# LPMP/BDD

Hardware: AMD Instinct MI355X
Metric: parallel-MMA iterations/sec, 10.5M BDD nodes, 1 GPU (+ achieved HBM GB/s in roofline) (higher is better)
Workload: dtype f32

## Files before the change

bdd_amd/capi.py:

```python
from __future__ import annotations

import ctypes as C
import os
import subprocess

_HERE = os.path.dirname(os.path.abspath(__file__))
LIB_PATH = os.path.abspath(os.environ["BDDMMA_LIB"]) if os.environ.get("BDDMMA_LIB") else os.path.join(_HERE, "csrc", "libbdd_mma_hip.so")

OK = 0
ERR_INVALID_ARGUMENT, ERR_INVALID_BDD, ERR_DEVICE, ERR_STATE, ERR_UNSUPPORTED, ERR_IO = -1, -2, -3, -4, -5, -6
F32, F64 = 0, 1
K_FORWARD_MM, K_BACKWARD_MM, K_FINISH_DELTA, K_OTHER, K_COUNT = 0, 1, 2, 3, 4


class Options(C.Structure):
    _fields_ = [("pack_width", C.c_uint32), ("wide_pack_width", C.c_uint32), ("deterministic", C.c_uint32),
                ("vars_per_bin", C.c_uint32), ("stage_cap", C.c_uint32), ("waves_per_block", C.c_uint32),
                ("keep_bdd_order", C.c_uint32), ("resident_sweeps", C.c_uint32), ("exchange_by_variable", C.c_uint32),
                ("variant_flags", C.c_uint32), ("pack_fill", C.c_uint32), ("pack_stagger", C.c_uint32)]


class LbfgsParams(C.Structure):
    _fields_ = [("history_size", C.c_int32), ("init_step_size", C.c_double), ("req_rel_lb_increase", C.c_double),
                ("step_size_decrease_factor", C.c_double), ("step_size_increase_factor", C.c_double)]
# ... 25 lines not shown
    "bddmma_last_error": (C.c_char_p, [_V]),
    "bddmma_nr_variables": (_U64, [_V]),
    "bddmma_nr_bdds": (_U64, [_V]),
    "bddmma_nr_layers": (_U64, [_V]),
    "bddmma_nr_bdd_nodes": (_U64, [_V]),
    "bddmma_nr_hops": (_U64, [_V]),
    "bddmma_nr_packs": (_U64, [_V]),
    "bddmma_solve_sweep_kind": (_I, [_V]),
    "bddmma_fused_small": (_I, [_V]),
    "bddmma_fused_small_learned": (_I, [_V]),
    "bddmma_fused_small_history": (_I, [_V]),
    "bddmma_fused_small_stop": (_I, [_V]),
    "bddmma_nontemporal_loads": (_I, [_V]),
    "bddmma_potentials_on_chip": (_I, [_V]),
    "bddmma_onchip_hops": (_I, [_V]),
    "bddmma_precision": (_I, [_V]),
    "bddmma_device": (_I, [_V]),
    "bddmma_num_bdds_per_var": (_I, [_V, _V]),
    "bddmma_layer_variables": (_I, [_V, _V]),
    "bddmma_layer_bdds": (_I, [_V, _V]),
    "bddmma_nodes_per_hop": (_I, [_V, _V]),
    "bddmma_layers_per_hop": (_I, [_V, _V]),
    "bddmma_update_costs": (_I, [_V, _V, _U64, _V, _U64, _I, _I]),
    "bddmma_set_cost": (_I, [_V, _D, _U64]),
    "bddmma_get_solver_costs": (_I, [_V, _V, _V, _V, _I]),
    "bddmma_set_solver_costs": (_I, [_V, _V, _V, _V, _I]),
    "bddmma_primal_objective_vec": (_I, [_V, _V, _I]),
    "bddmma_forward_run": (_I, [_V]),
    "bddmma_backward_run": (_I, [_V]),
    "bddmma_lower_bound": (_I, [_V, C.POINTER(_D)]),
# ... 70 lines not shown
    "bddmma_stream_signal": (_I, [_V, _V]),
    "bddmma_set_profiling": (_I, [_V, _I]),
    "bddmma_get_profile": (_I, [_V, C.POINTER(Profile)]),
    "bddmma_time_iterations": (_I, [_V, _D, _U64, C.POINTER(_D)]),
    "bddmma_time_kernel": (_I, [_V, _I, _U64, C.POINTER(_D)]),
    "bddmma_device_bytes": (_U64, [_V]),
    "bddmma_device_allocated_bytes": (_U64, [_V]),
    "bddmma_layout_create": (_I, [C.POINTER(_V), _V, _V, _U64, C.POINTER(Options)]),
    "bddmma_layout_create_for_chip": (_I, [C.POINTER(_V), _V, _V, _U64, C.POINTER(Options), _I, C.c_uint32, C.c_uint32]),
    "bddmma_layout_destroy": (None, [_V]),
    "bddmma_layout_size": (_U64, [_V, _I]),
    "bddmma_layout_copy": (_I, [_V, _I, _V]),
    "bddmma_layout_res2_records": (_I, [_V, _I, _V, _V, _V]),
    "bddmma_layout_stream_records": (_I, [_V, _I, _V, _V, _V]),
    "bddmma_layout_layer_records": (_I, [_V, _I, _V, _V, _V]),
    "bddmma_layout_seg_exchange": (_I, [_V, _I, _I, _V, _V, _V, _V]),
}

_I64P, _U64P = C.POINTER(C.c_int64), C.POINTER(C.c_uint64)
ILP_SIGNATURES = {
    "bddilp_last_error": (C.c_char_p, []),
    "bddilp_parse_lp": (_I, [C.c_char_p, C.POINTER(_V)]),
    "bddilp_parse_opb": (_I, [C.c_char_p, C.POINTER(_V)]),
    "bddilp_parse": (_I, [C.c_char_p, C.POINTER(_V)]),
    "bddilp_destroy": (None, [_V]),
    "bddilp_nr_variables": (_U64, [_V]),
    "bddilp_nr_constraints": (_U64, [_V]),
    "bddilp_variable_name": (C.c_char_p, [_V, _U64]),
    "bddilp_objective": (_I, [_V, _V, C.POINTER(_D)]),
    "bddilp_constraint_size": (_U64, [_V, _U64]),
# ... 53 lines not shown
```

bdd_amd/csrc/capi.cpp:

```cpp
#include <chrono>
#include <cmath>
#include <cstdio>
#include <cstdlib>
#include <cstring>
#include <limits>
#include <new>
#include <string>
#include <vector>

#include "../../include/bdd_mma.h"
#include "layout.hpp"
#include "solver.hpp"

using namespace bddmma;

struct bddmma_lbfgs;
extern "C" int bddmma_lbfgs_iteration(bddmma_lbfgs* l);
extern "C" int bddmma_lbfgs_update_costs(bddmma_lbfgs* l, const void* lo, uint64_t n_lo, const void* hi, uint64_t n_hi, int elem_precision,
                                         int on_device);

namespace {
thread_local std::string g_err;

template <typename F>
// ... 121 lines not shown

uint64_t bddmma_nr_variables(const bddmma_solver* s) { return s && s->impl ? s->impl->n_vars : 0; }
uint64_t bddmma_nr_bdds(const bddmma_solver* s) { return s && s->impl ? s->impl->n_bdds : 0; }
uint64_t bddmma_nr_layers(const bddmma_solver* s) { return s && s->impl ? s->impl->n_layers : 0; }
uint64_t bddmma_nr_bdd_nodes(const bddmma_solver* s) { return s && s->impl ? s->impl->n_input_nodes : 0; }
uint64_t bddmma_nr_hops(const bddmma_solver* s) { return s && s->impl ? s->impl->n_hops : 0; }
uint64_t bddmma_nr_packs(const bddmma_solver* s) { return s && s->impl ? s->impl->n_packs_narrow + s->impl->n_packs_wide : 0; }
int bddmma_solve_sweep_kind(const bddmma_solver* s) { return s && s->impl ? s->impl->solve_sweep_kind : -1; }
int bddmma_fused_small(const bddmma_solver* s) { return s && s->impl ? (s->impl->fused_small ? 1 : 0) : -1; }
int bddmma_fused_small_learned(const bddmma_solver* s) { return s && s->impl ? (s->impl->fused_small_learned ? 1 : 0) : -1; }
int bddmma_fused_small_history(const bddmma_solver* s) { return s && s->impl ? (s->impl->fused_small_history ? 1 : 0) : -1; }
int bddmma_fused_small_stop(const bddmma_solver* s) { return s && s->impl ? (s->impl->fused_small_stop ? 1 : 0) : -1; }
int bddmma_nontemporal_loads(const bddmma_solver* s) { return s && s->impl ? (s->impl->nt_loads ? 1 : 0) : -1; }
int bddmma_potentials_on_chip(const bddmma_solver* s) { return s && s->impl ? (s->impl->pot_on_chip ? 1 : 0) : -1; }
int bddmma_onchip_hops(const bddmma_solver* s) { return s && s->impl ? s->impl->onchip_hops : -1; }
int bddmma_precision(const bddmma_solver* s) { return s && s->impl ? s->impl->precision : -1; }
int bddmma_device(const bddmma_solver* s) { return s && s->impl ? s->impl->device : -1; }
uint64_t bddmma_device_bytes(const bddmma_solver* s) { return s && s->impl ? s->impl->dev_bytes : 0; }
uint64_t bddmma_device_allocated_bytes(const bddmma_solver* s) { return s && s->impl ? s->impl->dev_alloc_bytes : 0; }

int bddmma_num_bdds_per_var(const bddmma_solver* s, int32_t* out)
{
    return guarded(s, [&](SolverBase* b) { return copy_host(b->h_nbdds, out); });
}
int bddmma_layer_variables(const bddmma_solver* s, int32_t* out)
{
    return guarded(s, [&](SolverBase* b) { return copy_host(b->h_layer_var, out); });
}
int bddmma_layer_bdds(const bddmma_solver* s, int32_t* out)
{
// ... 786 lines not shown
    if (rec_off && !R.rec_off.empty()) std::memcpy(rec_off, R.rec_off.data(), R.rec_off.size() * sizeof(uint32_t));
    return BDDMMA_OK;
}

int bddmma_layout_layer_records(const bddmma_layout* l, int real_size, uint32_t* info, uint32_t* words, uint32_t* rec_off)
{
    if (!l || !info || (real_size != 4 && real_size != 8)) return BDDMMA_ERR_INVALID_ARGUMENT;
    LayerRecords R;
    build_layer_records(l->L, (uint32_t)real_size, R);
    info[0] = R.ok ? 1u : 0u; info[1] = (uint32_t)R.rec.size();
    if (words && !R.rec.empty()) std::memcpy(words, R.rec.data(), R.rec.size() * sizeof(uint32_t));
    if (rec_off && !R.rec_off.empty()) std::memcpy(rec_off, R.rec_off.data(), R.rec_off.size() * sizeof(uint32_t));
    return BDDMMA_OK;
}

}
```

bdd_amd/csrc/kernels.hpp:

```cpp
#pragma once
#include <hip/hip_runtime.h>

#include <cstdint>
#include <type_traits>

#include "layout.hpp"

#include "kernels/common.hpp"
#include "kernels/stream.hpp"
#include "kernels/narrow.hpp"
#include "kernels/resident.hpp"
#include "kernels/narrow2.hpp"
#include "kernels/narrow3.hpp"
#include "kernels/narrow4.hpp"
#include "kernels/wide.hpp"
#include "kernels/exchange.hpp"
#include "kernels/small.hpp"
#include "kernels/elementwise.hpp"
```

bdd_amd/csrc/layout.cpp:

```cpp
#include "layout.hpp"

#include <algorithm>
#include <atomic>
#include <chrono>
#include <cstdio>
#include <cstdlib>
#include <mutex>
#include <thread>
#include <unordered_map>
#include <cstring>
#include <limits>

namespace bddmma {

namespace {

std::atomic<unsigned> g_layout_threads{0};
thread_local unsigned t_layout_threads = 0;
struct Par {
    unsigned nt = 1;
    Par()
    {
        const char* e = std::getenv("BDDMMA_THREADS");
        const unsigned hw = std::thread::hardware_concurrency();
// ... 1562 lines not shown
                    ++l;
                } else {
                    if (pos != 1 || l == 0 || !(w & NW_TWO) || (r[4 * (l - 1) + 2] & 0xFFFFu) != (j - 1) * S) { out = LayerRecords(); return; }
                    const uint32_t k = l - 1;
                    r[4 * k + 1] = child(lo, k) | (child(hi, k) << 16);
                    r[4 * k + 2] |= LREC_TWO << 16;
                    r[4 * k + 3] = (r[4 * k + 3] & 0xFFFFu) | ((j * S) << 16);
                }
            }
            if (l != nl) { out = LayerRecords(); return; }
        }
    }
    out.ok = true;
}

void set_layout_threads(unsigned n) { g_layout_threads.store(n, std::memory_order_relaxed); }
void set_thread_layout_threads(unsigned n) { t_layout_threads = n; }

}
```

bdd_amd/csrc/layout.hpp:

```cpp
#pragma once
#include <cstdint>
#include <string>
#include <vector>

#include "../../include/bdd_mma.h"

#ifndef __host__
#define __host__
#define __device__
#endif

namespace bddmma {

constexpr uint32_t NW_CHILD_BITS = 9;
constexpr uint32_t NW_CHILD_MASK = (1u << NW_CHILD_BITS) - 1;
constexpr uint32_t NW_POS_SHIFT = 18, NW_LIDX_SHIFT = 24, NW_FIELD6 = 63;
constexpr uint32_t NW_TWO = 1u << 30;
constexpr uint32_t NW_PAD = 1u << 31;
constexpr uint32_t nw_top(uint32_t pack_width) { return pack_width; }
constexpr uint32_t nw_bot(uint32_t pack_width) { return pack_width + 1; }
constexpr uint32_t nw_pad_word(uint32_t pack_width)
{
    return NW_PAD | (nw_bot(pack_width) << NW_CHILD_BITS) | nw_bot(pack_width);
}
// ... 166 lines not shown
    bool ok = false;
    std::vector<uint32_t> rec;
    std::vector<uint32_t> rec_off;
};
void build_stream_records(const HostLayout& L, uint32_t real_size, StreamRecords& out);

constexpr uint32_t LREC_NO_STORE = 0xFFF0u;
constexpr uint32_t LREC_TWO = 1u, LREC_REAL = 2u;
struct LayerRecords {
    bool ok = false;
    std::vector<uint32_t> rec;
    std::vector<uint32_t> rec_off;
};
void build_layer_records(const HostLayout& L, uint32_t real_size, LayerRecords& out);

struct LinComb {
    const char* g;
    const void* S;
    const char* Y;
    uint64_t slot;
    const double* cy;
    const double* cs;
    const uint32_t* order;
    int ns;
};
constexpr int LINCOMB_MAX = 8;

struct SegExchange {
    bool ok = false;
    uint32_t threads = 0;
// ... 20 lines not shown
```

bdd_amd/csrc/solver.hpp:

```cpp
#pragma once
#include <hip/hip_runtime.h>

#include <cstdint>
#include <limits>
#include <memory>
#include <string>
#include <utility>
#include <vector>

#include "../../include/bdd_mma.h"
#include "layout.hpp"

namespace bddmma {

struct SolverBase {
    int precision = BDDMMA_F32, device = -1;
    hipStream_t stream = nullptr;
    std::string err;
    uint64_t n_vars = 0, n_bdds = 0, n_layers = 0, n_hops = 0, n_input_nodes = 0, n_slots = 0;
    int solve_sweep_kind = 0;
    uint32_t pack_width = 0, wide_pack_width = 0, wide_slot_base = 0;
    uint64_t dev_bytes = 0;
    uint64_t dev_alloc_bytes = 0;
    bool fwd_valid = false, bwd_valid = false;
// ... 34 lines not shown
        return BDDMMA_OK;
    }
    virtual int learned_iterations(const void* dist_weights, int weights_on_device, uint64_t num_itr, double omega, double improvement_slope,
                                   void* sol_avg, void* lb_first_diff_avg, void* lb_second_diff_avg, uint64_t compute_history_for_itr,
                                   double history_avg_beta, int outputs_on_device, uint64_t* itr_done, const void* omega_vec,
                                   int omega_vec_on_device) = 0;
    virtual int isotropic_dist_weights(void* out, int on_device) = 0;
    double initial_lb_change = std::numeric_limits<double>::infinity();
    std::shared_ptr<int> lbfgs_attached = std::make_shared<int>(0);
    bool fused_small = false;
    bool fused_small_learned = false;
    bool fused_small_history = false;
    bool fused_small_stop = false;
    bool nt_loads = false;
    bool pot_on_chip = false;
    int onchip_hops = 0;
    virtual int run_plain(uint64_t max_iter, double tolerance, double slope, double time_limit, int verbose, bddmma_run_result* res) = 0;
    virtual int forward_mm(double omega, void* delta, int on_device) = 0;
    virtual int backward_mm(double omega, void* delta, int on_device) = 0;
    virtual int normalize_delta(void* delta, int on_device) = 0;
    virtual int distribute_delta() = 0;
    virtual int get_delta(void* out, int on_device) = 0;
    virtual int set_delta(const void* in, int on_device) = 0;
    virtual int update_costs(const void* lo, uint64_t n_lo, const void* hi, uint64_t n_hi, int elem_precision, int on_device) = 0;
    virtual int set_cost(double c, uint64_t var) = 0;
    virtual int get_solver_costs(void* lo, void* hi, void* mm, int on_device) = 0;
    virtual int set_solver_costs(const void* lo, const void* hi, const void* mm, int on_device) = 0;
    virtual int primal_objective_vec(void* out, int on_device) = 0;
    virtual int min_marginals(int sorted, int32_t* var, void* mm0, void* mm1, int on_device) = 0;
    virtual int min_marginal_diff(void* out, int on_device) = 0;
// ... 92 lines not shown
```

bdd_amd/csrc/solver_impl.hpp:

```cpp
#pragma once
#include <hip/hip_runtime.h>
#include <atomic>
#include <chrono>
#include <cmath>
#include <cstdio>
#include <cstdlib>
#include <cstring>
#include <limits>
#include <memory>
#include <string>
#include <thread>
#include <type_traits>
#include <vector>
#include "../../include/bdd_mma.h"
#include "kernels.hpp"
#include "layout.hpp"
#include "solver.hpp"

namespace bddmma {

static inline void cpu_relax()
{
#if defined(__x86_64__) || defined(__i386__)
    __asm__ __volatile__("pause");
// ... 132 lines not shown
    int small_nw = 1;
    uint32_t small_lds = 0;
    SmallDev small{};
    uint32_t* d_small_lds = nullptr;
    bool small_ln_ok = false, small_ln_rl = false, sl_ready = false;
    bool small_stop_ok = false;
    bool small_hist_ok = false;
    uint32_t small_ln_lds = 0;
    SmallDev small_ln{};
    SmallLearn<REAL> small_ln_arg{};
    bool use_narrow3 = false;
    int onchip_hc = 0;
    uint32_t onchip_mode = 0;
    uint32_t *d_lrec = nullptr, *d_lrec_off = nullptr;
    uint32_t lrec_words = 0;
    uint32_t huge_pack_width = 0;
    unsigned char* d_huge_scratch = nullptr;

    std::vector<void*> allocs;

    ~SolverT() override
    {
        if (device >= 0) (void)hipSetDevice(device);
        for (void* p : allocs) (void)hipFree(p);
        if (h_lb) (void)hipHostFree(h_lb);
        if (h_lb_seq) (void)hipHostFree(h_lb_seq);
        if (h_run) (void)hipHostFree(h_run);
        if (d_run_ctl) (void)hipFree(d_run_ctl);
        for (auto& e : ev_pool) {
            (void)hipEventDestroy(e.first);
// ... 257 lines not shown
                const uint64_t in_flight = (uint64_t)n_cus * wgs2 * wpb;
                const bool auto_ok = sizeof(REAL) == 4 ? (uint64_t)nb_.n_packs * 100 <= in_flight * 145 : (uint64_t)nb_.n_packs <= in_flight;
                if (wgs2 && (mode == 2 || auto_ok)) {
                    Res2Records R2;
                    build_res2_records(L, sizeof(REAL), res2_ns, res2_nl, R2);
                    if (R2.ok && R2.rec.size() * sizeof(uint32_t) < (1ull << 31)) {
                        if ((rc = upload(&d_res2_rec, R2.rec))) return rc;
                        if ((rc = upload(&d_res2_rec_off, R2.rec_off))) return rc;
                        res2_n_words = (uint32_t)R2.rec.size();
                        use_res2 = use_res = true;
                    }
                }
            }
        }
        uint32_t narrow2_static = 0;
        if (nb_.n_packs && !use_res && !wb_.n_packs && !(opts && (opts->variant_flags & 0x1000u))) {
            StreamRecords SR;
            build_stream_records(L, sizeof(REAL), SR);
            narrow2_static = L.ex.waves_per_block * ((2 * pack_width + 2 + pack_width + 2) * (uint32_t)sizeof(REAL) + 3 * 64 * 4 + 64);
            const bool forced = opts && (opts->variant_flags & 0x2000u);
            const bool shared = forced || (SR.rec.size() * sizeof(uint32_t) <= (uint64_t)L.narrow_slots * sizeof(REAL) / 2 &&
                                           (sizeof(REAL) == 8 || n_slots <= 16'000'000ull));
            if (SR.ok && shared && stage_lds + narrow2_static + seg_bytes(L.ex.waves_per_block) <= 64 * 1024) {
                if ((rc = upload(&d_srec, SR.rec))) return rc;
                if ((rc = upload(&d_srec_off, SR.rec_off))) return rc;
                srec_words = (uint32_t)SR.rec.size();
                use_narrow2 = true;
                narrow_gen = narrow_seg;
                for (uint16_t r : L.narrow.hop_root) narrow_gen = narrow_gen || r != NO_ROOT;
            }
        }
        if (nb_.n_packs && !use_res && !wb_.n_packs && !hb_.n_packs && !narrow_seg && pack_width == 128 && (L.ex.waves_per_block == 4 || L.ex.waves_per_block == 8) &&
            !(opts && (opts->variant_flags & 0x41000u))) {
            LayerRecords LR;
            build_layer_records(L, sizeof(REAL), LR);
            const uint32_t n3_static = L.ex.waves_per_block * (4 * (128 + 128) * (uint32_t)sizeof(REAL) + 3 * 64 * 4);
            const bool forced = opts && (opts->variant_flags & 0x2000u);
            const bool shared = forced || (LR.rec.size() * sizeof(uint32_t) <= (uint64_t)L.narrow_slots * sizeof(REAL) / 2 && n_slots <= 16'000'000ull);
            if (LR.ok && shared && stage_lds + n3_static <= lds_cu - 1024) {
                if ((rc = upload(&d_lrec, LR.rec))) return rc;
                if ((rc = upload(&d_lrec_off, LR.rec_off))) return rc;
                lrec_words = (uint32_t)LR.rec.size();
                use_narrow3 = true;
                n3_nt = sizeof(REAL) == 8 && nt_potentials != 0;
            }
        }
        if (nb_.n_packs && !use_res && !use_narrow3 && !wb_.n_packs && !hb_.n_packs && !narrow_seg && !narrow_gen && pack_width == 128 &&
            (L.ex.waves_per_block == 4 || L.ex.waves_per_block == 8) && (beyond_cache || (opts && (opts->variant_flags & 0x100000u))))
#ifndef BDDMMA_EXP_NO_N12_NT
            n12_nt = !use_narrow2 || sizeof(REAL) == 8;
// ... 2 lines not shown
#endif
        nt_loads = n3_nt || n12_nt;
        if constexpr (sizeof(REAL) == 4) {
            if (use_narrow3 && res_hdr_ok && !n3_nt && !(opts && (opts->variant_flags & 0x200000u))) {
                uint32_t max_hops = 0;
                for (uint32_t p = 0; p < nb_.n_packs; ++p) max_hops = std::max(max_hops, L.res.pack_hdr[8 * (size_t)p + 5] & 0xFFFFu);
                onchip_hc = max_hops <= 10 ? 10 : max_hops <= 12 ? 12 : max_hops <= 16 ? 16 : 0;
                const uint32_t part = opts ? (opts->variant_flags >> 22) & 3u : 0u;
                if (onchip_hc == 16) onchip_mode = 3;
                if (part == 1 || part == 2) {
                    if (onchip_hc == 10 && wpb == 4) onchip_mode = part;
                    else onchip_hc = 0;
                }
                pot_on_chip = onchip_hc != 0;
                onchip_hops = onchip_hc;
            }
        }
        if (wb_.n_packs) {
            wide_threads = std::min<uint32_t>(1024, std::max<uint32_t>(64, ((wide_pack_width + 1) / 2 + 63) / 64 * 64));
            wide_npt = (wide_pack_width + wide_threads - 1) / wide_threads;
            wide_npt = wide_npt <= 1 ? 1 : (wide_npt <= 2 ? 2 : 4);
            wide_lds = (uint32_t)wide2_lds_bytes(sizeof(REAL), wide_pack_width, true);
            if (wide_lds > lds_cu || wide_pack_width > 4096) {
                err = "wide_pack_width " + std::to_string(wide_pack_width) + " needs " + std::to_string(wide_lds) + " B of LDS (> 160 KiB)";
                return BDDMMA_ERR_UNSUPPORTED;
            }
        }
        if (wb_.n_packs && nb_.n_packs && !use_res && !(opts && (opts->variant_flags & 1u))) {
            const uint32_t threads = 64 * wpb;
            const uint32_t npt = (wide_pack_width + threads - 1) / threads;
// ... 189 lines not shown
            if (mixed)
                s.mixed = {pick<64, 128, 256>(pack_width, [&](auto PW) {
                               return pick<1, 2, 4, 8>(wpb, [&](auto W) {
                                   return pick<1, 2, 4>(mixed_npt, [&](auto N) -> MixedFn {
                                       constexpr int R = PW.value / 64;
                                       return bwd ? &k_bwd_mixed<REAL, R, W.value, N.value, OV> : &k_fwd_mixed<REAL, R, W.value, N.value, OV>;
                                   });
                               });
                           }),
                           mixed_lds};
        }
        return s;
    }
    RecFn onchip_fn(bool bwd, bool rebuild, bool store) const
    {
        if (onchip_hc == 16) return pick<4, 8>(wpb, [&](auto W) -> RecFn { return &k_bwd_narrow4<REAL, W.value, 16, true, true>; });
        if (onchip_hc == 12)
            return pick<4, 8>(wpb, [&](auto W) -> RecFn {
                return bwd ? &k_bwd_narrow4<REAL, W.value, 12, true, false> : &k_fwd_narrow4<REAL, W.value, 12, true, false>;
            });
        if (rebuild && !store)
            return pick<4, 8>(wpb, [&](auto W) -> RecFn {
                return bwd ? &k_bwd_narrow4<REAL, W.value, 10, true, false> : &k_fwd_narrow4<REAL, W.value, 10, true, false>;
            });
        if (rebuild) return bwd ? &k_bwd_narrow4<REAL, 4, 10, true, true> : &k_fwd_narrow4<REAL, 4, 10, true, true>;
        return bwd ? &k_bwd_narrow4<REAL, 4, 10, false, false> : &k_fwd_narrow4<REAL, 4, 10, false, false>;
    }
    void resolve_kernels()
    {
        for (int bwd = 0; bwd < 2; ++bwd) {
            kern.sweep[bwd][FWD_PLAIN] = resolve_sweep<FWD_PLAIN, false>(bwd);
            kern.sweep[bwd][FWD_SOLVE] = resolve_sweep<FWD_SOLVE, false>(bwd);
            kern.sweep[bwd][FWD_SOLUTION] = resolve_sweep<FWD_SOLUTION, false>(bwd);
        }
        if (onchip_hc) {
            for (int bwd = 0; bwd < 2; ++bwd) {
                Sweep s = kern.sweep[bwd][FWD_SOLVE];
                if (onchip_mode == 3 && !bwd) { kern.onchip[0] = s; continue; }
                const bool rebuild = onchip_mode == 0 || (onchip_mode == 1) == !bwd;
                const bool store = onchip_mode != 0 && rebuild;
                if constexpr (sizeof(REAL) == 4) s.rec = onchip_fn(bwd, rebuild, onchip_mode == 3 || store);
                s.reads_pot = !rebuild;
                s.stores_pot = onchip_mode == 3 || store;
                kern.onchip[bwd] = s;
            }
        }
        kern.ex_threads = exch_small ? EXS_THREADS : exch_medium ? EXM_THREADS : EX_THREADS;
        pick<EXS_THREADS, EXM_THREADS, EX_THREADS>(kern.ex_threads, [&](auto T_) {
            constexpr int T = T_.value, U = T == EXS_THREADS ? EXS_UNROLL : T == EXM_THREADS ? EXM_UNROLL : EX_UNROLL,
                          N = T == EXS_THREADS ? EXS_NPT : T == EXM_THREADS ? EXM_NPT : EX_NPT;
            kern.ex[0] = {&k_exchange_reduce<REAL, BDDMMA_EX_ACC, EX_ITER, T, U, N, false>, exch_lds};
            kern.ex[1] = {&k_exchange_reduce<REAL, BDDMMA_EX_ACC, EX_ITER, T, U, N, true>, exch_lds};
            kern.ex_w = {&k_exchange_reduce<REAL, BDDMMA_EX_ACC, EX_ITER, T, U, N, false, true>, exch_lds};
            kern.project = {&k_project_entries<REAL, T>, vars_per_bin * (uint32_t)sizeof(double)};
            if (use_seg)
                pick<2, 4>(seg_groups <= 2 ? 2 : 4, [&](auto G) {
// ... 1265 lines not shown
```

bdd_amd/solver.py:

```python
from __future__ import annotations

import ctypes as C

import numpy as np

from . import capi
from .bdd_collection import BddCollection


def _ptr(a):
    return a.ctypes.data_as(C.c_void_p) if a is not None else None


def _is_dev(x):
    return hasattr(x, "data_ptr") and bool(getattr(x, "is_cuda", False))


def _dev_ptr(x, n, dtype):
    assert x.is_contiguous() and x.numel() >= n, "device buffer too small or not contiguous"
    assert x.element_size() == np.dtype(dtype).itemsize, "device buffer has the wrong element type"
    return C.c_void_p(x.data_ptr())


class bdd_hip_parallel_mma:
# ... 53 lines not shown
    def fused_small_learned(self) -> bool:
        return bool(self._L.bddmma_fused_small_learned(self._h))
    def fused_small_history(self) -> bool:
        return bool(self._L.bddmma_fused_small_history(self._h))
    def fused_small_stop(self) -> bool:
        return bool(self._L.bddmma_fused_small_stop(self._h))

    def nontemporal_loads(self) -> bool:
        return bool(self._L.bddmma_nontemporal_loads(self._h))

    def potentials_on_chip(self) -> bool:
        return bool(self._L.bddmma_potentials_on_chip(self._h))

    def onchip_hops(self) -> int:
        return int(self._L.bddmma_onchip_hops(self._h))
    def device(self) -> int:
        return int(self._L.bddmma_device(self._h))
    def device_bytes(self): return int(self._L.bddmma_device_bytes(self._h))
    def device_allocated_bytes(self): return int(self._L.bddmma_device_allocated_bytes(self._h))

    def nr_bdds(self, var=None):
        if var is None:
            return int(self._L.bddmma_nr_bdds(self._h))
        return int(self.get_num_bdds_per_var()[var])

    def get_num_bdds_per_var(self):
        out = np.zeros(self.nr_variables(), np.int32)
        self._ck(self._L.bddmma_num_bdds_per_var(self._h, _ptr(out)))
        return out

# ... 797 lines not shown
```

include/bdd_mma.h:

```cpp
#ifndef BDD_MMA_H
#define BDD_MMA_H

#include <stddef.h>
#include <stdint.h>

#ifdef __cplusplus
extern "C" {
#endif

#define BDDMMA_OK 0
#define BDDMMA_ERR_INVALID_ARGUMENT (-1)
#define BDDMMA_ERR_INVALID_BDD (-2)
#define BDDMMA_ERR_DEVICE (-3)
#define BDDMMA_ERR_STATE (-4)
#define BDDMMA_ERR_UNSUPPORTED (-5)
#define BDDMMA_ERR_IO (-6)

#define BDDMMA_F32 0
#define BDDMMA_F64 1

typedef struct bddmma_instruction {
    uint64_t lo;
    uint64_t hi;
    uint64_t index;
// ... 42 lines not shown
    BDDMMA_SWEEPS_MIXED = 1,
    BDDMMA_SWEEPS_STREAMING1 = 2,
    BDDMMA_SWEEPS_STREAMING2 = 3,
    BDDMMA_SWEEPS_STREAMING3 = 4,
    BDDMMA_SWEEPS_RESIDENT1 = 5,
    BDDMMA_SWEEPS_RESIDENT2 = 6
};
int bddmma_solve_sweep_kind(const bddmma_solver* s);
int bddmma_fused_small(const bddmma_solver* s);
int bddmma_fused_small_learned(const bddmma_solver* s);
int bddmma_fused_small_history(const bddmma_solver* s);
int bddmma_fused_small_stop(const bddmma_solver* s);
int bddmma_nontemporal_loads(const bddmma_solver* s);
int bddmma_potentials_on_chip(const bddmma_solver* s);
int bddmma_onchip_hops(const bddmma_solver* s);
int bddmma_precision(const bddmma_solver* s);
int bddmma_device(const bddmma_solver* s);
int bddmma_num_bdds_per_var(const bddmma_solver* s, int32_t* out);
int bddmma_layer_variables(const bddmma_solver* s, int32_t* out);
int bddmma_layer_bdds(const bddmma_solver* s, int32_t* out);
int bddmma_nodes_per_hop(const bddmma_solver* s, uint64_t* out);
int bddmma_layers_per_hop(const bddmma_solver* s, uint64_t* out);

int bddmma_update_costs(bddmma_solver* s, const void* lo, uint64_t n_lo, const void* hi, uint64_t n_hi,
                        int elem_precision, int on_device);
int bddmma_set_cost(bddmma_solver* s, double c, uint64_t var);
int bddmma_get_solver_costs(const bddmma_solver* s, void* lo, void* hi, void* deferred_mm_diff, int on_device);
int bddmma_set_solver_costs(bddmma_solver* s, const void* lo, const void* hi, const void* deferred_mm_diff, int on_device);
int bddmma_primal_objective_vec(bddmma_solver* s, void* out, int on_device);

// ... 159 lines not shown
int bddmma_time_kernel(bddmma_solver* s, int kind, uint64_t reps, double* ms);
uint64_t bddmma_device_bytes(const bddmma_solver* s);
uint64_t bddmma_device_allocated_bytes(const bddmma_solver* s);

typedef struct bddmma_layout bddmma_layout;
int bddmma_layout_create(bddmma_layout** out, const bddmma_instruction* instr, const uint64_t* bdd_delims,
                         uint64_t n_bdds, const bddmma_options* opts);
int bddmma_layout_create_for_chip(bddmma_layout** out, const bddmma_instruction* instr, const uint64_t* bdd_delims,
                                  uint64_t n_bdds, const bddmma_options* opts, int real_size, uint32_t n_cus, uint32_t lds_bytes_per_cu);
void bddmma_layout_destroy(bddmma_layout* l);
uint64_t bddmma_layout_size(const bddmma_layout* l, int what);
int bddmma_layout_copy(const bddmma_layout* l, int which, void* out);
int bddmma_layout_res2_records(const bddmma_layout* l, int real_size, uint32_t* info, uint32_t* words, uint32_t* rec_off);
int bddmma_layout_stream_records(const bddmma_layout* l, int real_size, uint32_t* info, uint32_t* words, uint32_t* rec_off);
int bddmma_layout_layer_records(const bddmma_layout* l, int real_size, uint32_t* info, uint32_t* words, uint32_t* rec_off);
int bddmma_layout_seg_exchange(const bddmma_layout* l, int threads, int real_size, uint32_t* info, uint32_t* bin, uint16_t* perm, uint32_t* thr);

#ifdef __cplusplus
}
#endif
#endif
```

Measured before the change: 9727.

## Add lane-code on-chip sweep kernels encoding per-lane child topology in compact bit codes

Adds a new narrow5 forward/backward kernel that replaces per-hop layer record tables with a compact 10-bit per-hop, per-lane code (packed three hops per 32-bit word, one 128-bit load per lane). Each code says whether a child is the next layer's node A/B, the top sink or the bottom sink. The kernels resolve children with bit-select arithmetic instead of LDS-indexed gathers. The host builds and deduplicates these codes, and the path is enabled only for f32 when on-chip hop counts are 10 or 12 in mode 0. It cuts record traffic and LDS indexing in exchange for extra ALU bit manipulation and more host-side layout complexity.

Result: faster. 9891 (median of 6 runs) (+1.7%).

```diff
diff --git a/bdd_amd/capi.py b/bdd_amd/capi.py
--- a/bdd_amd/capi.py
+++ b/bdd_amd/capi.py
@@ -63,6 +63,7 @@
     "bddmma_nontemporal_loads": (_I, [_V]),
     "bddmma_potentials_on_chip": (_I, [_V]),
     "bddmma_onchip_hops": (_I, [_V]),
+    "bddmma_lane_sweeps": (_I, [_V]),
     "bddmma_precision": (_I, [_V]),
     "bddmma_device": (_I, [_V]),
     "bddmma_num_bdds_per_var": (_I, [_V, _V]),
@@ -163,6 +164,7 @@
     "bddmma_layout_res2_records": (_I, [_V, _I, _V, _V, _V]),
     "bddmma_layout_stream_records": (_I, [_V, _I, _V, _V, _V]),
     "bddmma_layout_layer_records": (_I, [_V, _I, _V, _V, _V]),
+    "bddmma_layout_lane_codes": (_I, [_V, _I, _V, _V, _V]),
     "bddmma_layout_seg_exchange": (_I, [_V, _I, _I, _V, _V, _V, _V]),
 }
 
diff --git a/bdd_amd/csrc/capi.cpp b/bdd_amd/csrc/capi.cpp
--- a/bdd_amd/csrc/capi.cpp
+++ b/bdd_amd/csrc/capi.cpp
@@ -159,6 +159,7 @@
 int bddmma_nontemporal_loads(const bddmma_solver* s) { return s && s->impl ? (s->impl->nt_loads ? 1 : 0) : -1; }
 int bddmma_potentials_on_chip(const bddmma_solver* s) { return s && s->impl ? (s->impl->pot_on_chip ? 1 : 0) : -1; }
 int bddmma_onchip_hops(const bddmma_solver* s) { return s && s->impl ? s->impl->onchip_hops : -1; }
+int bddmma_lane_sweeps(const bddmma_solver* s) { return s && s->impl ? (s->impl->lane_sweeps ? 1 : 0) : -1; }
 int bddmma_precision(const bddmma_solver* s) { return s && s->impl ? s->impl->precision : -1; }
 int bddmma_device(const bddmma_solver* s) { return s && s->impl ? s->impl->device : -1; }
 uint64_t bddmma_device_bytes(const bddmma_solver* s) { return s && s->impl ? s->impl->dev_bytes : 0; }
@@ -975,4 +976,17 @@
     return BDDMMA_OK;
 }
 
-}
+int bddmma_layout_lane_codes(const bddmma_layout* l, int real_size, uint32_t* info, uint32_t* words, uint32_t* code_off)
+{
+    if (!l || !info || (real_size != 4 && real_size != 8)) return BDDMMA_ERR_INVALID_ARGUMENT;
+    LayerRecords R;
+    build_layer_records(l->L, (uint32_t)real_size, R);
+    LaneCodes K;
+    build_lane_codes(l->L, (uint32_t)real_size, R, K);
+    info[0] = K.ok ? 1u : 0u; info[1] = (uint32_t)K.words.size(); info[2] = K.affine ? 1u : 0u;
+    if (words && !K.words.empty()) std::memcpy(words, K.words.data(), K.words.size() * sizeof(uint32_t));
+    if (code_off && !K.code_off.empty()) std::memcpy(code_off, K.code_off.data(), K.code_off.size() * sizeof(uint32_t));
+    return BDDMMA_OK;
+}
+
+}
diff --git a/bdd_amd/csrc/kernels.hpp b/bdd_amd/csrc/kernels.hpp
--- a/bdd_amd/csrc/kernels.hpp
+++ b/bdd_amd/csrc/kernels.hpp
@@ -13,6 +13,7 @@
 #include "kernels/narrow2.hpp"
 #include "kernels/narrow3.hpp"
 #include "kernels/narrow4.hpp"
+#include "kernels/narrow5.hpp"
 #include "kernels/wide.hpp"
 #include "kernels/exchange.hpp"
 #include "kernels/small.hpp"
diff --git a/bdd_amd/csrc/kernels/narrow5.hpp b/bdd_amd/csrc/kernels/narrow5.hpp
--- /dev/null
+++ b/bdd_amd/csrc/kernels/narrow5.hpp
@@ -0,0 +1,261 @@
+#pragma once
+
+namespace bddmma {
+
+#ifndef BDDMMA_N5_WAVES
+#define BDDMMA_N5_WAVES 5
+#endif
+constexpr int n5_waves(int hc) { return hc <= 10 ? BDDMMA_N5_WAVES : 4; }
+
+__device__ __forceinline__ uint32_t lane_hop_code(const u4v& cw, int h) { return (cw[h / 3] >> (10 * (h % 3))) & 0x3FFu; }
+__device__ __forceinline__ u4v lane_codes_again(const u4v& cw)
+{
+    uint32_t a = cw[0], b = cw[1], c = cw[2], e = cw[3];
+    asm volatile("" : "+v"(a), "+v"(b), "+v"(c), "+v"(e));
+    return u4v{a, b, c, e};
+}
+__device__ __forceinline__ uint32_t lane_bit(uint32_t code, uint32_t bit) { return (uint32_t)__builtin_amdgcn_sbfe((int)code, bit, 1u); }
+__device__ __forceinline__ float lane_pick(uint32_t m, float a, float b)
+{
+    return __builtin_bit_cast(float, (m & __builtin_bit_cast(uint32_t, a)) | (~m & __builtin_bit_cast(uint32_t, b)));
+}
+__device__ __forceinline__ float lane_child(uint32_t code, uint32_t k, float ta, float tb)
+{
+    const uint32_t odd = lane_bit(code, k), snk = lane_bit(code, k + 1);
+    const float node = lane_pick(odd, tb, ta);
+    const float sink = __builtin_bit_cast(float, odd & 0x7F800000u);
+    return lane_pick(snk, sink, node);
+}
+__device__ __forceinline__ void lane_push(float& fa, float& fb, uint32_t code, float p0, float p1, float p2, float p3)
+{
+    const float INF = inf_v<float>();
+    const float pv[4] = {p0, p1, p2, p3};
+    fa = fb = INF;
+#pragma unroll
+    for (uint32_t k = 0; k < 4; ++k) {
+        const uint32_t odd = lane_bit(code, 2 * k), snk = lane_bit(code, 2 * k + 1);
+        fa = rmin(fa, lane_pick(odd | snk, INF, pv[k]));
+        fb = rmin(fb, lane_pick(odd & ~snk, pv[k], INF));
+    }
+}
+
+template <typename REAL, int WPB, int HC>
+__device__ __forceinline__ void fwd_narrow5_body(const DevPtrs<REAL>& d, const PackDev& pk, const uint32_t* __restrict__ lcode,
+                                                 const uint32_t* __restrict__ lcode_off, uint32_t lcode_words, REAL omega, uint32_t block_id)
+{
+    static_assert(HC + 1 <= (int)HOP_WIN, "one window of hop offsets has to hold the pack");
+    static_assert(HC <= (int)LCODE_HOPS, "a lane's code words hold LCODE_HOPS hops");
+    using P2 = typename Pair<REAL>::type;
+    extern __shared__ __attribute__((aligned(16))) unsigned char dyn_lds[];
+    P2* sD = reinterpret_cast<P2*>(dyn_lds);
+    __shared__ uint32_t sOffN_[WPB][HOP_WIN], sOffL_[WPB][HOP_WIN], sOffR_[WPB][HOP_WIN];
+    const uint32_t tid = threadIdx.x;
+    const int wave = __builtin_amdgcn_readfirstlane((int)(tid >> 6));
+    const int lane = tid & 63;
+    const uint32_t n_quads = (pk.n_packs + WPB - 1) / WPB;
+    const uint32_t quad = block_to_pack(block_id, n_quads, pk.xcd_chunk);
+    BDDMMA_EXIT_IF(quad >= n_quads, d)
+    const uint32_t p = quad * WPB + wave;
+    const bool has_pack = p < pk.n_packs;
+    const uint32_t* const hp = pk.hdr_pack + 8 * (size_t)(has_pack ? p : 0);
+    const uint32_t q0 = !has_pack ? 0 : hp[4];
+    const uint32_t hops = !has_pack ? 0 : (hp[5] & 0xFFFFu);
+    const uint32_t q1 = q0 + hops;
+    const uint32_t cbase = has_pack ? lcode_off[p] : 0;
+    const uint32_t c0_h = pk.hdr_quad[4 * (size_t)quad], cnt = pk.hdr_quad[4 * (size_t)quad + 1];
+    BDDMMA_STAMP(p, 0);
+    const REAL INF = inf_v<REAL>();
+    const uint32_t slot_first = !has_pack ? 0 : hp[0], l0 = !has_pack ? 0 : hp[2];
+    NarrowRs<REAL> rs(d);
+    rs.rebase_layers(d, l0);
+    uint32_t ent[STAGE_ITERS], esl[STAGE_ITERS];
+    stage_load_tables<REAL, WPB, BDDMMA_LD_TAB_AUX>(ent, esl, rs, c0_h, cnt, tid);
+    const REAL* const lohi_p = d.lohi + 2 * (size_t)l0;
+    const rsrc_t rc = make_rsrc(lcode, lcode_words);
+    HopWindow hw{sOffN_[wave], sOffL_[wave], sOffR_[wave], q0, q1, slot_first, l0};
+    uint32_t lb[HC + 1];
+    P2 L[HC];
+    P2 T[HC + 1];
+#pragma unroll
+    for (int i = 0; i < HC + 1; ++i) T[i] = P2{REAL(0), REAL(0)};
+    const uint32_t db = (uint32_t)wave * pk.stage_cap * (uint32_t)sizeof(P2);
+    hw.fill(pk, q0, lane);
+#pragma unroll
+    for (int i = 0; i < HC + 1; ++i) lb[i] = hw.layer_off(q0 + i);
+#pragma unroll
+    for (int h = 0; h < HC; ++h)
+        hop_load(L[h], rs.lohi, (uint32_t)h < hops ? (uint32_t)lane * (uint32_t)sizeof(P2) : OOB, lb[h] * (uint32_t)sizeof(P2));
+    u4v cw = __builtin_amdgcn_raw_buffer_load_b128(rc, (uint32_t)lane * 16u, cbase * 16u, 0);
+    {
+        REAL ta = REAL(0), tb = REAL(0);
+#pragma unroll
+        for (int h = HC - 1; h >= 1; --h) {
+            if ((uint32_t)h < hops) {
+                const uint32_t code = lane_hop_code(cw, h);
+                const REAL tla = lane_child(code, 0, ta, tb), tha = lane_child(code, 2, ta, tb);
+                const REAL tlb = lane_child(code, 4, ta, tb), thb = lane_child(code, 6, ta, tb);
+                const P2 c = L[h];
+                ta = rmin(c.y + tha, c.x + tla);
+                tb = rmin(c.y + thb, c.x + tlb);
+                T[h] = P2{ta, tb};
+            }
+        }
+        BDDMMA_STAMP(p, 5);
+    }
+    cw = lane_codes_again(cw);
+    stage_load_pairs<REAL, WPB>(sD, ent, esl, rs, cnt, tid);
+    if (WPB > 1) __syncthreads(); else wave_sync();
+    BDDMMA_STAMP(p, 1);
+    REAL fa = (lane_hop_code(cw, 0) & (LREC_REAL << 8)) ? REAL(0) : INF, fb = INF;
+#pragma unroll
+    for (int h = 0; h < HC; ++h) {
+        if ((uint32_t)h < hops) {
+            const uint32_t code = lane_hop_code(cw, h), flags = code >> 8;
+            const uint32_t lbh = lb[h], lbn = lb[h + 1];
+            const uint32_t stg = db + (lbh + (uint32_t)lane) * (uint32_t)sizeof(P2);
+            const P2 c = L[h];
+            const P2 tn = T[h + 1];
+            const REAL tla = lane_child(code, 0, tn.x, tn.y), tha = lane_child(code, 2, tn.x, tn.y);
+            const REAL tlb = lane_child(code, 4, tn.x, tn.y), thb = lane_child(code, 6, tn.x, tn.y);
+            const P2 dd = lds_ld<P2>(dyn_lds, stg);
+            const REAL m0 = rmin((fa + c.x) + tla, (fb + c.x) + tlb);
+            const REAL m1 = rmin((fa + c.y) + tha, (fb + c.y) + thb);
+            const REAL mm = mm_diff1(m0, m1, omega);
+            P2 nc;
+            nc.x = (c.x + min0(mm)) + dd.x;
+            nc.y = (c.y + min0_neg(mm)) + dd.y;
+            const rsrc_t rl = hop_rsrc(reinterpret_cast<const P2*>(lohi_p), lbh, lbn - lbh);
+            hop_store(nc, rl, (uint32_t)lane * (uint32_t)sizeof(P2), lbh * (uint32_t)sizeof(P2));
+            if (flags & LREC_REAL) lds_st<REAL>(dyn_lds, stg, mm);
+            const REAL p0 = fa + nc.x, p1 = fa + nc.y, p2 = fb + nc.x, p3 = fb + nc.y;
+            lane_push(fa, fb, code, p0, p1, p2, p3);
+        }
+    }
+    BDDMMA_STAMP(p, 3);
+    if (WPB > 1) __syncthreads(); else wave_sync();
+    BDDMMA_STAMP(p, 2);
+    stage_flush<REAL, WPB>(sD, ent, esl, rs, cnt, tid);
+    BDDMMA_STAMP(p, 4);
+}
+
+template <typename REAL, int WPB, int HC>
+__global__ void __launch_bounds__(64 * WPB) __attribute__((amdgpu_waves_per_eu(n5_waves(HC)))) k_fwd_narrow5(DevPtrs<REAL> d, PackDev pk, const uint32_t* __restrict__ lcode, const uint32_t* __restrict__ lcode_off,
+                                                          uint32_t lcode_words, REAL omega)
+{
+    fwd_narrow5_body<REAL, WPB, HC>(d, pk, lcode, lcode_off, lcode_words, omega, blockIdx.x);
+}
+
+template <typename REAL, int WPB, int HC>
+__device__ __forceinline__ void bwd_narrow5_body(const DevPtrs<REAL>& d, const PackDev& pk, const uint32_t* __restrict__ lcode,
+                                                 const uint32_t* __restrict__ lcode_off, uint32_t lcode_words, REAL omega, uint32_t block_id)
+{
+    static_assert(HC + 1 <= (int)HOP_WIN, "one window of hop offsets has to hold the pack");
+    static_assert(HC <= (int)LCODE_HOPS, "a lane's code words hold LCODE_HOPS hops");
+    using P2 = typename Pair<REAL>::type;
+    extern __shared__ __attribute__((aligned(16))) unsigned char dyn_lds[];
+    P2* sD = reinterpret_cast<P2*>(dyn_lds);
+    __shared__ uint32_t sOffN_[WPB][HOP_WIN], sOffL_[WPB][HOP_WIN], sOffR_[WPB][HOP_WIN];
+    const uint32_t tid = threadIdx.x;
+    const int wave = __builtin_amdgcn_readfirstlane((int)(tid >> 6));
+    const int lane = tid & 63;
+    const uint32_t n_quads = (pk.n_packs + WPB - 1) / WPB;
+    const uint32_t quad = block_to_pack(block_id, n_quads, pk.xcd_chunk);
+    BDDMMA_EXIT_IF(quad >= n_quads, d)
+    const uint32_t p = quad * WPB + wave;
+    const bool has_pack = p < pk.n_packs;
+    const uint32_t* const hp = pk.hdr_pack + 8 * (size_t)(has_pack ? p : 0);
+    const uint32_t q0 = !has_pack ? 0 : hp[4];
+    const uint32_t hops = !has_pack ? 0 : (hp[5] & 0xFFFFu);
+    const uint32_t q1 = q0 + hops;
+    const uint32_t cbase = has_pack ? lcode_off[p] : 0;
+    const uint32_t c0_h = pk.hdr_quad[4 * (size_t)quad], cnt = pk.hdr_quad[4 * (size_t)quad + 1];
+    BDDMMA_STAMP(p, 0);
+    const REAL INF = inf_v<REAL>();
+    const uint32_t slot_first = !has_pack ? 0 : hp[0], l0 = !has_pack ? 0 : hp[2];
+    NarrowRs<REAL> rs(d);
+    rs.rebase_layers(d, l0);
+    uint32_t ent[STAGE_ITERS], esl[STAGE_ITERS];
+    stage_load_tables<REAL, WPB, BDDMMA_LD_TAB_AUX>(ent, esl, rs, c0_h, cnt, tid);
+    const REAL* const lohi_p = d.lohi + 2 * (size_t)l0;
+    const rsrc_t rc = make_rsrc(lcode, lcode_words);
+    HopWindow hw{sOffN_[wave], sOffL_[wave], sOffR_[wave], q0, q1, slot_first, l0};
+    uint32_t lb[HC + 1];
+    P2 L[HC];
+    P2 F[HC];
+#pragma unroll
+    for (int i = 0; i < HC; ++i) F[i] = P2{INF, INF};
+    const uint32_t db = (uint32_t)wave * pk.stage_cap * (uint32_t)sizeof(P2);
+    hw.fill(pk, q0, lane);
+#pragma unroll
+    for (int i = 0; i < HC + 1; ++i) lb[i] = hw.layer_off(q0 + i);
+#pragma unroll
+    for (int h = 0; h < HC; ++h)
+        hop_load(L[h], rs.lohi, (uint32_t)h < hops ? (uint32_t)lane * (uint32_t)sizeof(P2) : OOB, lb[h] * (uint32_t)sizeof(P2));
+    u4v cw = __builtin_amdgcn_raw_buffer_load_b128(rc, (uint32_t)lane * 16u, cbase * 16u, 0);
+    {
+        REAL fa = (lane_hop_code(cw, 0) & (LREC_REAL << 8)) ? REAL(0) : INF, fb = INF;
+#pragma unroll
+        for (int h = 0; h < HC; ++h) {
+            if ((uint32_t)h < hops) {
+                const uint32_t code = lane_hop_code(cw, h);
+                if (h >= 1) F[h] = P2{fa, fb};
+                if ((uint32_t)h + 1 < hops) {
+                    const P2 c = L[h];
+                    const REAL p0 = fa + c.x, p1 = fa + c.y, p2 = fb + c.x, p3 = fb + c.y;
+                    lane_push(fa, fb, code, p0, p1, p2, p3);
+                }
+            }
+        }
+        BDDMMA_STAMP(p, 5);
+    }
+    cw = lane_codes_again(cw);
+    stage_load_pairs<REAL, WPB>(sD, ent, esl, rs, cnt, tid);
+    if (WPB > 1) __syncthreads(); else wave_sync();
+    BDDMMA_STAMP(p, 1);
+    REAL ta = REAL(0), tb = REAL(0);
+#pragma unroll
+    for (int h = HC - 1; h >= 0; --h) {
+        if ((uint32_t)h < hops) {
+            const uint32_t code = lane_hop_code(cw, h), flags = code >> 8;
+            const uint32_t lbh = lb[h], lbn = lb[h + 1];
+            const uint32_t stg = db + (lbh + (uint32_t)lane) * (uint32_t)sizeof(P2);
+            const P2 c = L[h];
+            const REAL tla = lane_child(code, 0, ta, tb), tha = lane_child(code, 2, ta, tb);
+            const REAL tlb = lane_child(code, 4, ta, tb), thb = lane_child(code, 6, ta, tb);
+            const P2 dd = lds_ld<P2>(dyn_lds, stg);
+            const REAL fa = h >= 1 ? F[h].x : (flags & LREC_REAL) ? REAL(0) : INF;
+            const REAL fb = h >= 1 ? F[h].y : INF;
+            const REAL m0 = rmin((fa + c.x) + tla, (fb + c.x) + tlb);
+            const REAL m1 = rmin((fa + c.y) + tha, (fb + c.y) + thb);
+            const REAL mm = mm_diff1(m0, m1, omega);
+            P2 nc;
+            nc.x = (c.x + min0(mm)) + dd.x;
+            nc.y = (c.y + min0_neg(mm)) + dd.y;
+            ta = rmin(nc.y + tha, nc.x + tla);
+            tb = rmin(nc.y + thb, nc.x + tlb);
+            const rsrc_t rl = hop_rsrc(reinterpret_cast<const P2*>(lohi_p), lbh, lbn - lbh);
+            hop_store(nc, rl, (uint32_t)lane * (uint32_t)sizeof(P2), lbh * (uint32_t)sizeof(P2));
+            if (flags & LREC_REAL) lds_st<REAL>(dyn_lds, stg, mm);
+        }
+    }
+    BDDMMA_STAMP(p, 3);
+    if (WPB > 1) __syncthreads(); else wave_sync();
+    BDDMMA_STAMP(p, 2);
+    stage_flush<REAL, WPB>(sD, ent, esl, rs, cnt, tid);
+    BDDMMA_STAMP(p, 4);
+    if (!has_pack) return;
+    const uint32_t n0 = lb[1] - lb[0];
+    double s = 0.0;
+    if ((uint32_t)lane < n0) s += (double)ta;
+    for (int off2 = 32; off2 > 0; off2 >>= 1) s += __shfl_down(s, off2);
+    if (lane == 0) d.lb_partial[pk.lb_base + p] = s;
+}
+
+template <typename REAL, int WPB, int HC>
+__global__ void __launch_bounds__(64 * WPB) __attribute__((amdgpu_waves_per_eu(n5_waves(HC)))) k_bwd_narrow5(DevPtrs<REAL> d, PackDev pk, const uint32_t* __restrict__ lcode, const uint32_t* __restrict__ lcode_off,
+                                                          uint32_t lcode_words, REAL omega)
+{
+    bwd_narrow5_body<REAL, WPB, HC>(d, pk, lcode, lcode_off, lcode_words, omega, blockIdx.x);
+}
+
+}
diff --git a/bdd_amd/csrc/layout.cpp b/bdd_amd/csrc/layout.cpp
--- a/bdd_amd/csrc/layout.cpp
+++ b/bdd_amd/csrc/layout.cpp
@@ -1600,6 +1600,66 @@
     out.ok = true;
 }
 
+void build_lane_codes(const HostLayout& L, uint32_t S, const LayerRecords& R, LaneCodes& out)
+{
+    out = LaneCodes();
+    const PackSet& N = L.narrow;
+    const uint32_t P = N.n_packs(), W = L.pack_width;
+    if (!R.ok || R.rec_off.size() != P) return;
+    std::unordered_map<uint32_t, uint32_t> seen;
+    std::vector<uint32_t> words, code_off(P, 0);
+    bool fits = true;
+    for (uint32_t p = 0; p < P; ++p) {
+        const uint32_t q0 = N.pack_hop_ptr[p], nh = N.pack_hop_ptr[p + 1] - q0;
+        const auto it = seen.find(R.rec_off[p]);
+        if (it != seen.end()) { code_off[p] = it->second; continue; }
+        const uint32_t first = (uint32_t)(words.size() / 4);
+        seen.emplace(R.rec_off[p], first);
+        code_off[p] = first;
+        words.resize(words.size() + 64 * 4, 0u);
+        if (nh > LCODE_HOPS) fits = false;
+        if (nh && N.hop_node_off[q0 + 1] - N.hop_node_off[q0] != N.hop_layer_off[q0 + 1] - N.hop_layer_off[q0]) return;
+        const uint32_t* rec = &R.rec[(size_t)R.rec_off[p] * 4];
+        for (uint32_t h = 0; h < nh; ++h) {
+            const uint32_t* r = rec + (size_t)h * 64 * 4;
+            const uint32_t* rn = h + 1 < nh ? r + 64 * 4 : nullptr;
+            for (uint32_t l = 0; l < 64; ++l) {
+                const uint32_t top = (W + 2 * l) * S, bot = top + S;
+                const uint32_t flags = r[4 * l + 2] >> 16;
+                const bool real = flags & LREC_REAL, two = flags & LREC_TWO;
+                if (two && !real) return;
+                if (h == 0 && real && (two || (r[4 * l + 2] & 0xFFFFu) != l * S)) return;
+                const uint32_t nflags = rn ? rn[4 * l + 2] >> 16 : 0u;
+                const uint32_t na = (nflags & LREC_REAL) ? rn[4 * l + 2] & 0xFFFFu : 0xFFFFFFFFu;
+                const uint32_t nb = (nflags & LREC_REAL) && (nflags & LREC_TWO) ? na + S : 0xFFFFFFFFu;
+                uint32_t code = flags << 8;
+                for (uint32_t k = 0; k < 4; ++k) {
+                    const uint32_t off = (r[4 * l + k / 2] >> (16 * (k & 1))) & 0xFFFFu;
+                    const bool present = real && (k < 2 || two);
+                    uint32_t c;
+                    if (!present) {
+                        if (off != bot) return;
+                        c = LCODE_BOT;
+                    } else if (off == top) c = LCODE_TOP;
+                    else if (off == bot) c = LCODE_BOT;
+                    else if (off == na) c = LCODE_A;
+                    else if (off == nb) c = LCODE_B;
+                    else return;
+                    code |= c << (2 * k);
+                }
+                if (h < LCODE_HOPS) words[(size_t)(first + l) * 4 + h / 3] |= code << (10 * (h % 3));
+            }
+        }
+        for (uint32_t h = nh; h < LCODE_HOPS; ++h)
+            for (uint32_t l = 0; l < 64; ++l) words[(size_t)(first + l) * 4 + h / 3] |= 0xFFu << (10 * (h % 3));
+    }
+    out.affine = true;
+    if (!fits || (uint64_t)words.size() * 4 >= (1ull << 31)) return;
+    out.words.swap(words);
+    out.code_off.swap(code_off);
+    out.ok = true;
+}
+
 void set_layout_threads(unsigned n) { g_layout_threads.store(n, std::memory_order_relaxed); }
 void set_thread_layout_threads(unsigned n) { t_layout_threads = n; }
 
diff --git a/bdd_amd/csrc/layout.hpp b/bdd_amd/csrc/layout.hpp
--- a/bdd_amd/csrc/layout.hpp
+++ b/bdd_amd/csrc/layout.hpp
@@ -204,6 +204,16 @@
 };
 void build_layer_records(const HostLayout& L, uint32_t real_size, LayerRecords& out);
 
+constexpr uint32_t LCODE_A = 0u, LCODE_B = 1u, LCODE_TOP = 2u, LCODE_BOT = 3u;
+constexpr uint32_t LCODE_HOPS = 12;
+struct LaneCodes {
+    bool ok = false;
+    bool affine = false;
+    std::vector<uint32_t> words;
+    std::vector<uint32_t> code_off;
+};
+void build_lane_codes(const HostLayout& L, uint32_t real_size, const LayerRecords& R, LaneCodes& out);
+
 struct LinComb {
     const char* g;
     const void* S;
diff --git a/bdd_amd/csrc/solver.hpp b/bdd_amd/csrc/solver.hpp
--- a/bdd_amd/csrc/solver.hpp
+++ b/bdd_amd/csrc/solver.hpp
@@ -72,6 +72,7 @@
     bool fused_small_stop = false;
     bool nt_loads = false;
     bool pot_on_chip = false;
+    bool lane_sweeps = false;
     int onchip_hops = 0;
     virtual int run_plain(uint64_t max_iter, double tolerance, double slope, double time_limit, int verbose, bddmma_run_result* res) = 0;
     virtual int forward_mm(double omega, void* delta, int on_device) = 0;
diff --git a/bdd_amd/csrc/solver_impl.hpp b/bdd_amd/csrc/solver_impl.hpp
--- a/bdd_amd/csrc/solver_impl.hpp
+++ b/bdd_amd/csrc/solver_impl.hpp
@@ -170,6 +170,9 @@
     uint32_t onchip_mode = 0;
     uint32_t *d_lrec = nullptr, *d_lrec_off = nullptr;
     uint32_t lrec_words = 0;
+    bool lane5 = false;
+    uint32_t *d_lcode = nullptr, *d_lcode_off = nullptr;
+    uint32_t lcode_words = 0;
     uint32_t huge_pack_width = 0;
     unsigned char* d_huge_scratch = nullptr;
 
@@ -457,6 +460,7 @@
             }
         }
         uint32_t narrow2_static = 0;
+        LaneCodes lane_codes;
         if (nb_.n_packs && !use_res && !wb_.n_packs && !(opts && (opts->variant_flags & 0x1000u))) {
             StreamRecords SR;
             build_stream_records(L, sizeof(REAL), SR);
@@ -477,6 +481,7 @@
             !(opts && (opts->variant_flags & 0x41000u))) {
             LayerRecords LR;
             build_layer_records(L, sizeof(REAL), LR);
+            if constexpr (sizeof(REAL) == 4) build_lane_codes(L, sizeof(REAL), LR, lane_codes);
             const uint32_t n3_static = L.ex.waves_per_block * (4 * (128 + 128) * (uint32_t)sizeof(REAL) + 3 * 64 * 4);
             const bool forced = opts && (opts->variant_flags & 0x2000u);
             const bool shared = forced || (LR.rec.size() * sizeof(uint32_t) <= (uint64_t)L.narrow_slots * sizeof(REAL) / 2 && n_slots <= 16'000'000ull);
@@ -509,6 +514,12 @@
                 }
                 pot_on_chip = onchip_hc != 0;
                 onchip_hops = onchip_hc;
+                if ((onchip_hc == 10 || onchip_hc == 12) && onchip_mode == 0 && lane_codes.ok && !(opts && (opts->variant_flags & 0x1000000u))) {
+                    if ((rc = upload(&d_lcode, lane_codes.words))) return rc;
+                    if ((rc = upload(&d_lcode_off, lane_codes.code_off))) return rc;
+                    lcode_words = (uint32_t)lane_codes.words.size();
+                    lane5 = lane_sweeps = true;
+                }
             }
         }
         if (wb_.n_packs) {
@@ -728,6 +739,11 @@
     }
     RecFn onchip_fn(bool bwd, bool rebuild, bool store) const
     {
+        if (lane5)
+            return pick<4, 8>(wpb, [&](auto W) -> RecFn {
+                if (onchip_hc == 12) return bwd ? &k_bwd_narrow5<REAL, W.value, 12> : &k_fwd_narrow5<REAL, W.value, 12>;
+                return bwd ? &k_bwd_narrow5<REAL, W.value, 10> : &k_fwd_narrow5<REAL, W.value, 10>;
+            });
         if (onchip_hc == 16) return pick<4, 8>(wpb, [&](auto W) -> RecFn { return &k_bwd_narrow4<REAL, W.value, 16, true, true>; });
         if (onchip_hc == 12)
             return pick<4, 8>(wpb, [&](auto W) -> RecFn {
@@ -754,6 +770,7 @@
                 const bool rebuild = onchip_mode == 0 || (onchip_mode == 1) == !bwd;
                 const bool store = onchip_mode != 0 && rebuild;
                 if constexpr (sizeof(REAL) == 4) s.rec = onchip_fn(bwd, rebuild, onchip_mode == 3 || store);
+                if (lane5) { s.rec_tab = d_lcode; s.rec_off = d_lcode_off; s.rec_words = lcode_words; }
                 s.reads_pot = !rebuild;
                 s.stores_pot = onchip_mode == 3 || store;
                 kern.onchip[bwd] = s;
diff --git a/bdd_amd/solver.py b/bdd_amd/solver.py
--- a/bdd_amd/solver.py
+++ b/bdd_amd/solver.py
@@ -91,6 +91,8 @@
 
     def onchip_hops(self) -> int:
         return int(self._L.bddmma_onchip_hops(self._h))
+    def lane_sweeps(self) -> bool:
+        return bool(self._L.bddmma_lane_sweeps(self._h))
     def device(self) -> int:
         return int(self._L.bddmma_device(self._h))
     def device_bytes(self): return int(self._L.bddmma_device_bytes(self._h))
diff --git a/include/bdd_mma.h b/include/bdd_mma.h
--- a/include/bdd_mma.h
+++ b/include/bdd_mma.h
@@ -80,6 +80,7 @@
 int bddmma_nontemporal_loads(const bddmma_solver* s);
 int bddmma_potentials_on_chip(const bddmma_solver* s);
 int bddmma_onchip_hops(const bddmma_solver* s);
+int bddmma_lane_sweeps(const bddmma_solver* s);
 int bddmma_precision(const bddmma_solver* s);
 int bddmma_device(const bddmma_solver* s);
 int bddmma_num_bdds_per_var(const bddmma_solver* s, int32_t* out);
@@ -269,6 +270,7 @@
 int bddmma_layout_res2_records(const bddmma_layout* l, int real_size, uint32_t* info, uint32_t* words, uint32_t* rec_off);
 int bddmma_layout_stream_records(const bddmma_layout* l, int real_size, uint32_t* info, uint32_t* words, uint32_t* rec_off);
 int bddmma_layout_layer_records(const bddmma_layout* l, int real_size, uint32_t* info, uint32_t* words, uint32_t* rec_off);
+int bddmma_layout_lane_codes(const bddmma_layout* l, int real_size, uint32_t* info, uint32_t* words, uint32_t* code_off);
 int bddmma_layout_seg_exchange(const bddmma_layout* l, int threads, int real_size, uint32_t* info, uint32_t* bin, uint16_t* perm, uint32_t* thr);
 
 #ifdef __cplusplus
```
